# ArchDD/CPP-Raytracer-Rasterizer

Hardware: AMD Instinct MI355X
Metric: Mrays/s (primary+shadow) (higher is better)
Workload: dtype f32

## Files before the change

cpp-raytracer-rasterizer_amd/capi/binned.cpp:

```cpp
#include "capi.hpp"

namespace mirt {


int ensure_pairs(RtScratch &S, size_t cap)
{
    int r;
    if ((r = dev_realloc(&S.d_entries, cap)) || (r = dev_realloc(&S.d_pair_keys, cap)) || (r = dev_realloc(&S.d_pair_vals, cap)) ||
        (r = dev_realloc(&S.d_sorted_keys, cap)) || (r = dev_realloc(&S.d_tmp_vals, cap))) { S.cap_entries = 0; return r; }
    S.cap_entries = (uint32_t)cap;
    return MIRT_OK;
}

constexpr uint32_t BIN_MAX_KEYS = BUCKET_SORT_MAX_BUCKETS * 1024u - 1u;

void poll_pair_count(RtScratch &S)
{
    if (S.count_pending && hipEventQuery(S.ev_count) == hipSuccess) {
        S.known_pairs = *S.h_count; S.have_known = true; S.count_pending = false;
    }
    (void)hipGetLastError();
}

int bin_pass(RtScratch &S, BinSet bs, const OriginRow *cam_tab, const OriginRow *light_tab, uint32_t *counter, uint32_t *bin_off,
             bool fresh, uint32_t *npairs, bool may_guess = false)
{
    int rc;
    poll_pair_count(S);
    if (!fresh && may_guess && S.have_known && S.known_pairs > S.cap_used) fresh = true;
    const bool guess = fresh && may_guess && S.have_known;
    if (!S.d_entries || !S.cap_entries) {
        static const size_t initial = [] { const long v = env_int("MIRT_BIN_INITIAL_PAIRS", 0); return v > 0 ? (size_t)v : (size_t)1 << 20; }();
        if ((rc = ensure_pairs(S, initial))) return rc;
    }
    if (bs.nbins > BIN_MAX_KEYS) return fail(MIRT_ERR_INVALID_ARGUMENT, "binning: %u sort keys exceed the %u the bucket sort holds", bs.nbins, BIN_MAX_KEYS);
    bs.chunk_tris = 256;
    const dim3 bin_grid((unsigned)std::min<long long>((long long)((g.n + bs.chunk_tris - 1) / bs.chunk_tris) * bs.nframes, (long long)g.cu_count * 8));
    bs.counters = counter;
    const uint32_t nbuckets = bucket_sort_buckets(bs.nbins);
    if (nbuckets + 1 > S.cap_buckets) {
        S.cap_buckets = 0;
        if ((rc = dev_realloc(&S.d_bucket, (size_t)3 * (nbuckets + 1)))) return rc;
        HIP_TRY(hipMemsetAsync(S.d_bucket, 0, sizeof(uint32_t) * 3 * (nbuckets + 1), g.stream));
        S.cap_buckets = nbuckets + 1;
        S.bucket_dirty = false;
    }
    uint32_t *bcnt = S.d_bucket, *bbase = S.d_bucket + S.cap_buckets, *bcur = S.d_bucket + 2 * (size_t)S.cap_buckets;
    bs.bucket_cnt = bcnt; bs.nbuckets = nbuckets; bs.bucket_shift = bucket_sort_shift(bs.nbins);
    const size_t bin_lds = (size_t)nbuckets * sizeof(uint32_t);
    {
        static const bool once = [] {
            (void)hipFuncSetAttribute(reinterpret_cast<const void *>(&k_bin_pairs<512>), hipFuncAttributeMaxDynamicSharedMemorySize, 48 * 1024);
// ... 328 lines not shown
    const uint32_t cam_keys = (uint32_t)bs.frame0.nbu * (uint32_t)band_tile_rows * (uint32_t)bs.frame0.nshell;
    const int tshells = transient ? light_shells_for(nlights, cube_bins, 0u) : 1;
    const uint32_t per_light = 6u * (uint32_t)(cube_bins * cube_bins) * (uint32_t)tshells;
    bs.nbins = cam_keys;
    if (bs.nbins + 1 > S.cap_bins) {
        const size_t cap = (size_t)bs.nbins + 1;
        HIP_TRY(hipStreamSynchronize(g.stream));
        if ((rc = dev_realloc(&S.d_bin_off, cap))) { S.cap_bins = 0; return rc; }
        S.cap_bins = (uint32_t)cap;
        S.bin_key_valid = false;
    }
    if (!S.d_bin_counters) { HIP_TRY(hipMalloc(reinterpret_cast<void **>(&S.d_bin_counters), 512)); HIP_TRY(hipMemsetAsync(S.d_bin_counters, 0, 512, g.stream)); }
    if (S.sel_n != g.n) {
        HIP_TRY(hipStreamSynchronize(g.stream));
        S.sel_n = 0;
        if ((rc = dev_realloc(&S.d_sel, (size_t)g.n))) return rc;
        S.sel_n = g.n;
        S.bin_key_valid = false;
    }
    bs.bin_off = S.d_bin_off;

    uint64_t key = 0xcbf29ce484222325ull ^ g.scene_version;
    {
        auto mix = [&](const void *p, size_t nb) { const unsigned char *b = (const unsigned char *)p; for (size_t i = 0; i < nb; i++) { key ^= b[i]; key *= 0x100000001b3ull; } };
        mix(view, sizeof *view); mix(&y0, 4); mix(&y1, 4); mix(&g.n, 4); mix(&g.aa, 4);
    }
    const int bin_mode = 0;
    StreamState &ss = g.cur();
    ss.hits_clean[ss.hits_tog] = false;
    if (!S.d_frames) HIP_TRY(hipMalloc(reinterpret_cast<void **>(&S.d_frames), sizeof(BinFrameDesc) * (1 + 6 * MIRT_MAX_LIGHTS)));
    poll_pair_count(S);
// ... 20 lines not shown
        rc = transient_light_pass(L, f, origins, nlights, cube_bins, tshells, per_light, lkey, &lights_kept, reuse ? g.d_hits : nullptr);
        g.stream = main_stream;
        if (rc) return rc;
        if (forked) HIP_TRY(hipEventRecord(ss.ev_join, ss.aux));
    }
    if (reuse) {
        if (!(transient && !lights_kept)) HIP_TRY(hipMemsetAsync(g.d_hits, 0, HIT_BYTES, g.stream));
        g.stats.bins_reused = 1;
    } else {
        S.sel_parity ^= 1;
        SelectOut so;
        memset(&so, 0, sizeof so);
        so.cam_tab = S.d_cam_tab; so.sel = S.d_sel;
        so.sel_count = S.d_bin_counters + SEL_COUNT0 + S.sel_parity; so.sel_count_next = S.d_bin_counters + SEL_COUNT0 + (S.sel_parity ^ 1);
        so.zero_hits = g.d_hits; so.zero_counter = S.d_bin_counters;
        if ((rc = hist_prepare(S, bs.frame0, &so))) return rc;
        const unsigned sel_grid = (unsigned)std::min<long long>(((long long)g.n + 1023) / 1024, (long long)g.cu_count);
        hipLaunchKernelGGL(k_prep_select, dim3(sel_grid), dim3(1024), 0, g.stream, g.d_tris, g.n, bs.frame0, so);
        if ((rc = hist_publish(S))) return rc;
        bs.sel = S.d_sel; bs.sel_count = so.sel_count;
        g.stats_sel_count = so.sel_count;
        if ((rc = bin_pass(S, bs, S.d_cam_tab, nullptr, S.d_bin_counters, S.d_bin_off, true, &S.bin_entries, may_guess))) return rc;
        S.last_bin_mode = bin_mode;
        S.bin_key = key;
        S.bin_key_valid = true;
        if ((size_t)order_seg > S.cap_order) {
            HIP_TRY(hipStreamSynchronize(g.stream));
            S.cap_order = 0;
            if ((rc = dev_realloc(&S.d_order, (size_t)ORDER_GROUPS * ORDER_CLASSES * order_seg))) return rc;
            S.cap_order = order_seg;
        }
        hipLaunchKernelGGL(k_tile_order, dim3((pairs_x + 63) / 64, (unsigned)(bs.frame0.j1 - bs.frame0.j0)), dim3(64), 0, g.stream, cam_off, bs.frame0.nshell,
                           bs.frame0.nbu, bs.frame0.j0, bs.frame0.j1, S.d_bin_counters, S.cap_used, S.d_order, order_seg);
    }
    if (forked) HIP_TRY(hipStreamWaitEvent(g.stream, ss.ev_join, 0));
// ... 10 lines not shown
}

int hist_only_pass(const mirt_view *view)
{
    int rc;
    g.stream = g.cur().stream;
    RtScratch &S = g.cur().rt;
    if (S.cam_tab_n != g.n) {
        S.cam_tab_n = 0;
        if ((rc = dev_realloc(&S.d_cam_tab, (size_t)g.n))) return rc;
        S.cam_tab_n = g.n;
    }
    if (S.sel_n != g.n) {
        HIP_TRY(hipStreamSynchronize(g.stream));
        S.sel_n = 0;
        if ((rc = dev_realloc(&S.d_sel, (size_t)g.n))) return rc;
        S.sel_n = g.n;
    }
    if (!S.d_bin_counters) { HIP_TRY(hipMalloc(reinterpret_cast<void **>(&S.d_bin_counters), 512)); HIP_TRY(hipMemsetAsync(S.d_bin_counters, 0, 512, g.stream)); }
    S.bin_key_valid = false;
    const BinFrameDesc fr = make_camera_frame(view, 0, 0, g.aa);
    SelectOut so;
    memset(&so, 0, sizeof so);
    so.cam_tab = S.d_cam_tab; so.sel = S.d_sel;
    so.sel_count = S.d_bin_counters + HIST_SEL_COUNT; so.sel_count_next = S.d_bin_counters + HIST_SEL_COUNT + 1;
    if ((rc = hist_prepare(S, fr, &so))) return rc;
    if (!g.hist_armed) return MIRT_OK;
    HIP_TRY(hipMemsetAsync(so.sel_count, 0, 4, g.stream));
    const unsigned sel_grid = (unsigned)std::min<long long>(((long long)g.n + 1023) / 1024, (long long)g.cu_count);
    if (sel_grid) hipLaunchKernelGGL(k_prep_select, dim3(sel_grid), dim3(1024), 0, g.stream, g.d_tris, g.n, fr, so);
    HIP_TRY(hipGetLastError());
// ... 59 lines not shown
```

cpp-raytracer-rasterizer_amd/capi/capi.hpp:

```cpp
#pragma once

#include "../csrc/bin_sort.hpp"
#include "../csrc/comm.hpp"
#include "../csrc/cull.hpp"
#include "../csrc/dof.hpp"
#include "../csrc/rt_common.hpp"
#include "../csrc/raster_common.hpp"
#include "../csrc/rt_binned.hpp"
#include "../csrc/scan.hpp"
#include "env.hpp"

#include <cstdarg>
#include <cstdio>
#include <cstdlib>
#include <cstring>
#include <algorithm>
#include <cmath>
#include <vector>

#define MIRT_KERNEL __attribute__((global))

namespace mirt {

MIRT_KERNEL void k_prep_origin(const float *, int, const float *, v3, int, OriginRow *, OriginRow *, uint32_t *, unsigned long long *, uint32_t *);
// ... 49 lines not shown

extern char g_err[512];
int fail(int code, const char *fmt, ...);

#define HIP_TRY(expr)                                                                          \
    do {                                                                                       \
        hipError_t e_ = (expr);                                                                \
        if (e_ != hipSuccess)                                                                  \
            return fail(MIRT_ERR_HIP, "%s failed: %s (%s:%d)", #expr, hipGetErrorString(e_), __FILE__, __LINE__); \
    } while (0)

enum { EV_CALL0 = 0, EV_CALL1 = 1, EV_K0 = 2, EV_COUNT = 2 + 2 * 8 };
constexpr int MAX_FLIGHT = 4;
constexpr int SEL_COUNT0 = 80;
constexpr int HIST_SEL_COUNT = 82;
constexpr int HIST_RING = 4;
constexpr int HIST_SLOTS = HIST_RING + 1;
constexpr size_t HIT_BYTES = sizeof(unsigned long long) * HIT_SHARDS * HIT_SHARD_STRIDE;

struct RtScratch {
    OriginRow *d_cam_tab = nullptr;
    OriginRow *d_light_tab = nullptr;
    int cam_tab_n = 0, light_tab_n = 0, light_tab_lights = 0;
    float *d_origins = nullptr;
    uint32_t *d_flags = nullptr;
    BinFrameDesc *d_frames = nullptr;
    uint32_t *d_bin_off = nullptr, *d_bin_counters = nullptr;
    uint32_t *d_entries = nullptr;
    uint32_t *d_pair_keys = nullptr, *d_pair_vals = nullptr, *d_sorted_keys = nullptr;
    uint32_t *d_tmp_vals = nullptr;
// ... 279 lines not shown
```

cpp-raytracer-rasterizer_amd/csrc/rt_binned.hip:

```cpp
#include "rt_binned.hpp"

#include <float.h>

namespace mirt {

constexpr int BIN_L0 = BIN_COARSE * BIN_COARSE;

struct BinItem {
    float A0[4], A1[4], A2[4], Bu[4], Bv[4];
    float lou, hiu, lov, hiv;
};

__device__ __forceinline__ float bcastf(float v, int lane) { return __builtin_bit_cast(float, __builtin_amdgcn_readlane(__builtin_bit_cast(int, v), lane)); }

__device__ __forceinline__ float corner(float s, float lo, float hi) { return fmaxf(s * lo, s * hi); }

__device__ __forceinline__ bool cell_may_hit(const BinItem &u, const float (&A)[4], float I, float J, float K)
{
    bool ok = true;
#pragma unroll
    for (int k = 0; k < 4; k++) ok = ok && (__builtin_fmaf(J, u.Bv[k], __builtin_fmaf(I, u.Bu[k], A[k])) >= 0.0f);
    return ok && (I + K >= u.lou) && (I <= u.hiu) && (J + K >= u.lov) && (J <= u.hiv);
}

// ... 23 lines not shown
    for (int i = 0; i < 4; i++)
#pragma unroll
        for (int j = i + 1; j < 4; j++) {
#pragma unroll
            for (int k = j + 1; k < 4; k++) empty = empty || bin_triple_infeasible(G[i], G[j], G[k], U, V);
#pragma unroll
            for (int sd = 0; sd < 4; sd++) empty = empty || bin_triple_infeasible(G[i], G[j], side[sd], U, V);
        }
    return empty;
}

struct BinFrameGrid { int nbu, fj0, fj1, cells_x, cy0, ncell; uint32_t fbase, nshell; };

constexpr int BIN_PAIR_BUF = 4096;
constexpr int BIN_TESTS_PER_THREAD = 2;
constexpr int BIN_DIRECT_SIDE = 32;

struct BinLargeSink {
    uint32_t *s_keys, *s_vals;
    uint32_t *s_fill;
    uint32_t *s_valid;
    uint32_t *g_count;
    BinPairs out;
    uint32_t *bucket_cnt;
    int bucket_shift;
};

__device__ __forceinline__ void bin_walk_large(const BinItem &u, uint32_t utri, uint32_t ushell, const BinFrameGrid &gr, int lane,
                                               const BinLargeSink &sink, unsigned long long cells0)
{
// ... 45 lines not shown
            }
        }
    }
#ifdef MIRT_BIN_STATS
    if (lane == 0) {
        uint32_t *c = sink.g_count;
        atomicAdd(&c[2], 1u); atomicAdd(&c[3], dbg_l1); atomicAdd(&c[4], dbg_steps); atomicAdd(&c[5], dbg_pairs);
        atomicMax(&c[6], dbg_steps);
        if (dbg_steps > 100) atomicAdd(&c[7], 1u);
    }
#endif
}

constexpr int SEL_WG = 1024;
constexpr int SEL_STAGE = 8192;

__global__ __launch_bounds__(SEL_WG) void k_prep_select(const float *__restrict__ tris15, int n, const BinFrameDesc fr, const SelectOut out)
{
    __shared__ uint32_t s_hist[SEL_HIST_MAX];
    __shared__ uint32_t s_sel[SEL_STAGE];
    __shared__ uint32_t s_fill, s_base;
    const int lane = threadIdx.x & 63;
    if (blockIdx.x == 0) {
        if (out.zero_hits)
            for (int g = threadIdx.x; g < HIT_SHARDS * HIT_SHARD_STRIDE; g += SEL_WG) out.zero_hits[g] = 0ull;
        if (out.zero_counter && (threadIdx.x == 0 || (threadIdx.x >= 16 && threadIdx.x < 80))) out.zero_counter[threadIdx.x] = 0u;
        if (threadIdx.x == 0) *out.sel_count_next = 0u;
        if (out.zero_faces && (int)threadIdx.x < out.zero_faces_n) out.zero_faces[threadIdx.x] = 0u;
    }
    if (out.hist && threadIdx.x < SEL_HIST_MAX) s_hist[threadIdx.x] = 0u;
    if (threadIdx.x == 0) s_fill = 0u;
    __syncthreads();
    const v3 S = V3(fr.S[0], fr.S[1], fr.S[2]);
    const int nchunks = (n + SEL_WG - 1) / SEL_WG;
    const int hist_rows = ((fr.nbv - 1) >> out.hist_shift) + 1;
    auto flush = [&]() {
        __syncthreads();
        const uint32_t staged = s_fill;
        if (threadIdx.x == 0 && staged) s_base = atomicAdd(out.sel_count, staged);
        __syncthreads();
        const uint32_t base = s_base;
        for (uint32_t i = threadIdx.x; i < staged; i += SEL_WG) out.sel[base + i] = s_sel[i];
        __syncthreads();
        if (threadIdx.x == 0) s_fill = 0u;
        __syncthreads();
    };
    for (int c = blockIdx.x; c < nchunks; c += gridDim.x) {
        if (s_fill + (uint32_t)SEL_WG > (uint32_t)SEL_STAGE) flush();
        const int i = c * SEL_WG + (int)threadIdx.x;
        bool keep = false;
        OriginRow r;
        if (i < n) {
            const float *t15 = tris15 + (size_t)15 * i;
            r = make_origin_row(t15, S);
            PreBox box;
            bool boxed;
            keep = frame_may_see(r, ld3(t15), ld3(t15 + 3), ld3(t15 + 6), fr, &box, &boxed);
            if (out.hist && boxed) {
                const float flo_u = fmaxf(ceilf(box.lou) - 1.0f, 0.0f), fhi_u = fminf(floorf(box.hiu), (float)(fr.nbu - 1));
                const float flo_v = fmaxf(ceilf(box.lov) - 1.0f, 0.0f), fhi_v = fminf(floorf(box.hiv), (float)(fr.nbv - 1));
                if (flo_u <= fhi_u && flo_v <= fhi_v) {
                    const uint32_t wi = (uint32_t)((int)fhi_u - (int)flo_u + 1);
                    const int ja = (int)flo_v, jb = (int)fhi_v;
                    for (int cr = ja >> out.hist_shift; cr <= (jb >> out.hist_shift) && cr < hist_rows; cr++) {
                        const int lo = max(ja, cr << out.hist_shift), hi = min(jb, ((cr + 1) << out.hist_shift) - 1);
                        atomicAdd(&s_hist[cr], wi * (uint32_t)(hi - lo + 1));
                    }
                }
            }
            if (keep) out.cam_tab[i] = r;
        }
        const unsigned long long m = __builtin_amdgcn_ballot_w64(keep);
        if (m) {
            uint32_t at0 = 0;
            if (lane == 0) at0 = atomicAdd(&s_fill, (uint32_t)__popcll(m));
            at0 = (uint32_t)__builtin_amdgcn_readfirstlane((int)at0);
            if (keep) s_sel[at0 + (uint32_t)__popcll(m & ((1ull << lane) - 1ull))] = (uint32_t)i;
        }
        __syncthreads();
    }
    flush();
    if (out.hist && threadIdx.x < SEL_HIST_MAX) {
        const uint32_t v = s_hist[threadIdx.x];
        if (v && (int)threadIdx.x < hist_rows) atomicAdd(&out.hist[threadIdx.x], v);
    }
}

constexpr int FACE_STAGE = 2048;
__global__ __launch_bounds__(SEL_WG) void k_select_faces(const float *__restrict__ tris15, int n, const float *__restrict__ origins ,
                                                        const BinFrameDesc *__restrict__ faces , OriginRow *__restrict__ light_tab,
                                                        uint32_t *__restrict__ lists, uint32_t stride, uint32_t *__restrict__ face_counts)
{
// ... 58 lines not shown
                                                   const OriginRow *__restrict__ light_tab, int n, BinSet bs, BinPairs out)
{
    extern __shared__ uint32_t s_bucket[];
    __shared__ uint32_t s_keys[BIN_PAIR_BUF], s_vals[BIN_PAIR_BUF];
    __shared__ float4 s_A2[256], s_Bu[256], s_Bv[256], s_box[256];
    __shared__ uint32_t s_org[256];
    __shared__ uint32_t s_ni[256];
    __shared__ uint32_t s_tri[256];
    __shared__ uint32_t s_pre[257];
    __shared__ uint32_t s_wave[4];
    __shared__ uint32_t s_base, s_fill, s_valid;
    const int lane = threadIdx.x & 63, wave = threadIdx.x >> 6;
    const int chunk_tris = bs.chunk_tris;
    const int nchunks = (n + chunk_tris - 1) / chunk_tris;
    const bool listed = bs.sel != nullptr;
    const uint32_t nsel = listed ? min(*bs.sel_count, (uint32_t)n) : 0u;
    const int cam_chunk = (listed && nsel < 32768u) ? 64 : chunk_tris;
    const int ncam = listed ? (int)((nsel + (uint32_t)cam_chunk - 1u) / (uint32_t)cam_chunk) : 0;
    const int nrest = listed ? bs.nframes - 1 : bs.nframes;
    const bool faces_listed = bs.face_lists != nullptr;
    __shared__ uint32_t s_first[MAX_BIN_FRAMES + 1];
    if (faces_listed) {
        if (threadIdx.x == 0) {
            uint32_t run = 0;
            for (int ff = 0; ff < nrest; ff++) { s_first[ff] = run; run += (min(bs.face_counts[ff], (uint32_t)n) + (uint32_t)chunk_tris - 1u) / (uint32_t)chunk_tris; }
            s_first[nrest] = run;
        }
        __syncthreads();
    }
    const int nwork = ncam + (faces_listed ? (int)s_first[nrest] : nchunks * nrest);
    if (threadIdx.x == 0) { s_fill = 0u; s_valid = (uint32_t)BIN_PAIR_BUF; }
    if (bs.bucket_cnt)
        for (uint32_t b = threadIdx.x; b < bs.nbuckets; b += WG) s_bucket[b] = 0u;
// ... 34 lines not shown
        int chunk, frame;
        const uint32_t *list = nullptr;
        uint32_t nhere = (uint32_t)n;
        const bool from_cam_list = w < ncam;
        if (from_cam_list) { chunk = w; frame = 0; list = bs.sel; nhere = nsel; }
        else if (faces_listed) {
            const uint32_t w2 = (uint32_t)(w - ncam);
            int lo = 0, hi = nrest;
            while (hi - lo > 1) { const int mid = (lo + hi) >> 1; if (s_first[mid] <= w2) lo = mid; else hi = mid; }
            chunk = (int)(w2 - s_first[lo]);
            frame = lo + (listed ? 1 : 0);
            list = bs.face_lists + (size_t)lo * bs.face_stride;
            nhere = min(bs.face_counts[lo], (uint32_t)n);
        } else { const int w2 = w - ncam; chunk = w2 / nrest; frame = w2 - chunk * nrest + (listed ? 1 : 0); }
        const int item_tris = from_cam_list ? cam_chunk : chunk_tris;
        const uint32_t slot = (uint32_t)chunk * (uint32_t)item_tris + threadIdx.x;
        const uint32_t tri = ((int)threadIdx.x < item_tris && slot < nhere) ? (list ? list[slot] : slot) : 0xFFFFFFFFu;
        const BinFrameDesc fr = bs.frames ? bs.frames[frame] : bs.frame0;
        BinFrameGrid gr;
        gr.nbu = fr.nbu; gr.fj0 = fr.j0; gr.fj1 = fr.j1; gr.fbase = fr.base; gr.nshell = (uint32_t)max(fr.nshell, 1);
        gr.cells_x = (gr.nbu + BIN_L0 - 1) / BIN_L0; gr.cy0 = gr.fj0 / BIN_L0;
        gr.ncell = gr.cells_x * ((gr.fj1 + BIN_L0 - 1) / BIN_L0 - gr.cy0);
        const int nbu = gr.nbu, fj0 = gr.fj0, fj1 = gr.fj1;
        BinItem it;
        memset(&it, 0, sizeof it);
        int kind = 0;
#ifdef MIRT_BIN_STATS
        int dbg_state = 0;
#endif
        int i_lo = 0, i_hi = -1, j_lo = 0, j_hi = -1;
        unsigned long long cells = 0;
        uint32_t shell = 0;
        if (tri < (uint32_t)n && fj1 > fj0) {
            const OriginRow &row = (fr.tab == 0) ? cam_tab[tri] : light_tab[(size_t)(fr.tab - 1) * n + tri];
            shell = bin_shell_of(fr, row.r1.w);
            TriBinFns t = make_bin_fns(row, fr);
            add_bbox(t, tris15 + (size_t)15 * tri, fr);
#ifdef MIRT_BIN_STATS
// ... 3 lines not shown
            const bool both = fabsf(t.nb) < T || !(t.nb == t.nb);
            const float sgn = t.nb < 0.0f ? -1.0f : 1.0f;
            const EdgeFn *fn[4] = { &t.n, &t.p, &t.q, &t.s };
            const float inf = __builtin_huge_valf();
#pragma unroll
            for (int k = 0; k < 4; k++) {
                const float su = sgn * fn[k]->cu, sv = sgn * fn[k]->cv;
                const float base = sgn * fn[k]->c0 + fn[k]->m + su * fr.ulo + sv * fr.vlo;
                it.Bu[k] = both ? 0.0f : su * fr.du;
                it.Bv[k] = both ? 0.0f : sv * fr.dv;
                it.A0[k] = both ? inf : base + corner(su, fr.pad_lo, (float)BIN_L0 * fr.du + fr.pad_hi) + corner(sv, fr.pad_lo, (float)BIN_L0 * fr.dv + fr.pad_hi);
                it.A1[k] = both ? inf : base + corner(su, fr.pad_lo, (float)BIN_COARSE * fr.du + fr.pad_hi) + corner(sv, fr.pad_lo, (float)BIN_COARSE * fr.dv + fr.pad_hi);
                it.A2[k] = both ? inf : base + corner(su, fr.pad_lo, fr.du + fr.pad_hi) + corner(sv, fr.pad_lo, fr.dv + fr.pad_hi);
            }
            if (t.bstate == BOX_VALID) {
                it.lou = (t.bu0 - fr.ulo - fr.pad_hi) / fr.du; it.hiu = (t.bu1 - fr.ulo - fr.pad_lo) / fr.du;
                it.lov = (t.bv0 - fr.vlo - fr.pad_hi) / fr.dv; it.hiv = (t.bv1 - fr.vlo - fr.pad_lo) / fr.dv;
                it.lou -= 3.814697265625e-06f * (1.0f + fabsf(it.lou)); it.hiu += 3.814697265625e-06f * (1.0f + fabsf(it.hiu));
                it.lov -= 3.814697265625e-06f * (1.0f + fabsf(it.lov)); it.hiv += 3.814697265625e-06f * (1.0f + fabsf(it.hiv));
            } else if (t.bstate == BOX_EMPTY) {
                it.lou = it.lov = inf; it.hiu = it.hiv = -inf;
            } else {
                it.lou = it.lov = -inf; it.hiu = it.hiv = inf;
            }
            const float flo_u = fmaxf(ceilf(it.lou) - 1.0f, 0.0f), fhi_u = fminf(floorf(it.hiu), (float)(nbu - 1));
            const float flo_v = fmaxf(ceilf(it.lov) - 1.0f, (float)fj0), fhi_v = fminf(floorf(it.hiv), (float)(fj1 - 1));
            if (flo_u <= fhi_u && flo_v <= fhi_v) {
                i_lo = (int)flo_u; i_hi = (int)fhi_u; j_lo = (int)flo_v; j_hi = (int)fhi_v;
                kind = (i_hi - i_lo < BIN_DIRECT_SIDE && j_hi - j_lo < BIN_DIRECT_SIDE) ? 1 : 2;
            }
            if (kind == 2) {
                for (int c = 0; c < gr.ncell && c < 64; c++) {
                    const int cx = c % gr.cells_x, cy = gr.cy0 + c / gr.cells_x;
                    if (cell_may_hit(it, it.A0, (float)(cx * BIN_L0), (float)(cy * BIN_L0), (float)BIN_L0)) cells |= 1ull << c;
// ... 140 lines not shown
```

cpp-raytracer-rasterizer_amd/csrc/rt_binned.hpp:

```cpp
#pragma once

#include "rt_common.hpp"

namespace mirt {

#ifndef MIRT_ORDER_STRIPE_SHIFT
#define MIRT_ORDER_STRIPE_SHIFT 2
#endif
constexpr int ORDER_STRIPE_SHIFT = MIRT_ORDER_STRIPE_SHIFT;
constexpr int BIN_TILE = 8;
constexpr int BIN_COARSE = 8;
constexpr int CUBE_BINS_MIN = 64;
constexpr int MAX_BIN_FRAMES = 1 + 6 * MIRT_MAX_LIGHTS;

struct BinFrameDesc {
    float P0[3], Pu[3], Pv[3];
    float S[3];
    float ru[3], rv[3], rw[3];
    float ulo, vlo, du, dv;
    float pad_lo, pad_hi;
    float dmax;
    int nbu, nbv;
    int j0, j1;
    uint32_t base;
// ... 16 lines not shown
struct BinSet {
    const BinFrameDesc *frames;
    BinFrameDesc frame0;
    int nframes;
    uint32_t nbins;
    uint32_t *bin_off;
    uint32_t *entries;
    uint32_t cap_entries;
    uint32_t *counters;
    uint32_t *bucket_cnt;
    uint32_t nbuckets;
    int bucket_shift;
    int chunk_tris;
    const uint32_t *sel;
    const uint32_t *sel_count;
    const uint32_t *face_lists;
    const uint32_t *face_counts;
    uint32_t face_stride;
};

constexpr int SEL_HIST_MAX = 256;
struct SelectOut {
    OriginRow *cam_tab;
    uint32_t *sel;
    uint32_t *sel_count;
    uint32_t *sel_count_next;
    uint32_t *hist;
    int hist_shift;
    uint32_t *zero_faces;
    int zero_faces_n;
    unsigned long long *zero_hits;
    uint32_t *zero_counter;
};

struct BinPairs {
    uint32_t *keys;
    uint32_t *vals;
    uint32_t cap;
};

struct EdgeFn { float c0, cu, cv, m; };

__device__ __forceinline__ EdgeFn make_edge_fn(float gx, float gy, float gz, const BinFrameDesc &fr)
{
    EdgeFn e;
    e.c0 = gx * fr.P0[0] + gy * fr.P0[1] + gz * fr.P0[2];
    e.cu = gx * fr.Pu[0] + gy * fr.Pu[1] + gz * fr.Pu[2];
// ... 28 lines not shown

__device__ __forceinline__ void add_bbox(TriBinFns &t, const float *t15, const BinFrameDesc &fr)
{
    float us[3], vs[3], pad = 0.0f;
    int front = 0, behind = 0;
#pragma unroll
    for (int j = 0; j < 3; j++) {
        const float gx = fr.S[0] - t15[3 * j], gy = fr.S[1] - t15[3 * j + 1], gz = fr.S[2] - t15[3 * j + 2];
        const float w = fr.rw[0] * gx + fr.rw[1] * gy + fr.rw[2] * gz;
        const float wm = fabsf(fr.rw[0] * gx) + fabsf(fr.rw[1] * gy) + fabsf(fr.rw[2] * gz);
        front += (w > 0.00390625f * wm);
        behind += (w < -0.00390625f * wm);
        const float un = fr.ru[0] * gx + fr.ru[1] * gy + fr.ru[2] * gz, vn = fr.rv[0] * gx + fr.rv[1] * gy + fr.rv[2] * gz;
        const float um = fabsf(fr.ru[0] * gx) + fabsf(fr.ru[1] * gy) + fabsf(fr.ru[2] * gz);
        const float vm = fabsf(fr.rv[0] * gx) + fabsf(fr.rv[1] * gy) + fabsf(fr.rv[2] * gz);
        us[j] = un / w; vs[j] = vn / w;
        const float iw = 1.0f / fabsf(w);
        pad = fmaxf(pad, 4.76837158203125e-07f * ((um + fabsf(us[j]) * wm) * iw + (vm + fabsf(vs[j]) * wm) * iw) +
                             2.384185791015625e-07f * (fabsf(us[j]) + fabsf(vs[j])));
    }
    if (front != 3 && behind != 3) return;
    const float u0 = fminf(fminf(us[0], us[1]), us[2]), u1 = fmaxf(fmaxf(us[0], us[1]), us[2]);
    const float v0 = fminf(fminf(vs[0], vs[1]), vs[2]), v1 = fmaxf(fmaxf(vs[0], vs[1]), vs[2]);
    const float ext = fmaxf(u1 - u0, v1 - v0);
    const float ax = us[1] - us[0], ay = vs[1] - vs[0], bx = us[2] - us[0], by = vs[2] - vs[0], cx = us[2] - us[1], cy = vs[2] - vs[1];
    const float area2 = fabsf(ax * by - ay * bx);
    const float per = sqrtf(ax * ax + ay * ay) + sqrtf(bx * bx + by * by) + sqrtf(cx * cx + cy * cy);
    const float dp = t.p.m / sqrtf(t.p.cu * t.p.cu + t.p.cv * t.p.cv);
    const float dq = t.q.m / sqrtf(t.q.cu * t.q.cu + t.q.cv * t.q.cv);
    const float ds = t.s.m / sqrtf(t.s.cu * t.s.cu + t.s.cv * t.s.cv);
    const float d = fmaxf(fmaxf(dp, dq), ds) + pad;
    if (behind == 3) {
        const float area_lo = area2 - 2.0f * pad * per - 4.76837158203125e-07f * (fabsf(ax * by) + fabsf(ay * bx));
        if (d < 0.5f * (area_lo / per)) t.bstate = BOX_EMPTY;
        return;
    }
    const float l01 = sqrtf(ax * ax + ay * ay), l02 = sqrtf(bx * bx + by * by), l12 = sqrtf(cx * cx + cy * cy);
    const float e01x = ax / l01, e01y = ay / l01, e02x = bx / l02, e02y = by / l02, e12x = cx / l12, e12y = cy / l12;
    const float dd = 1.25f * d;
    const float k0 = dd / fabsf(e01x * e02y - e01y * e02x), k1 = dd / fabsf(e01x * e12y - e01y * e12x), k2 = dd / fabsf(e02x * e12y - e02y * e12x);
    const float px0 = us[0] - k0 * (e01x + e02x), py0 = vs[0] - k0 * (e01y + e02y);
    const float px1 = us[1] - k1 * (e12x - e01x), py1 = vs[1] - k1 * (e12y - e01y);
    const float px2 = us[2] + k2 * (e02x + e12x), py2 = vs[2] + k2 * (e02y + e12y);
    const float slack = 2.0f * pad + 1.0e-6f * ext;
    const float bu0 = fminf(fminf(px0, px1), px2) - slack, bu1 = fmaxf(fmaxf(px0, px1), px2) + slack;
    const float bv0 = fminf(fminf(py0, py1), py2) - slack, bv1 = fmaxf(fmaxf(py0, py1), py2) + slack;
    if (!(bu0 > -1.0e30f && bu1 < 1.0e30f && bv0 > -1.0e30f && bv1 < 1.0e30f)) return;
    t.bu0 = fminf(bu0, u0 - slack); t.bu1 = fmaxf(bu1, u1 + slack); t.bv0 = fminf(bv0, v0 - slack); t.bv1 = fmaxf(bv1, v1 + slack);
    t.bstate = BOX_VALID;
}

struct PreBox { float lou, hiu, lov, hiv; };
__device__ __forceinline__ bool frame_may_see(const OriginRow &row, v3 va, v3 vb, v3 vc, const BinFrameDesc &fr, PreBox *box, bool *boxed)
{
    *boxed = false;
    const float nbv = row.r0.w;
    if (!(fabsf(nbv) >= 1.6940658945086007e-21f)) return true;
    const v3 vert[3] = { va, vb, vc };
    float us[3], vs[3], pad = 0.0f;
// ... 99 lines not shown
```

cpp-raytracer-rasterizer_amd/csrc/rt_trace.hip:

```cpp
#include "rt_binned.hpp"

#include <float.h>

namespace mirt {


__global__ __launch_bounds__(256) void k_geo_table(const float *__restrict__ tris15, int n, GeoRow *__restrict__ geo, ShadeRow *__restrict__ shade)
{
    const int t = blockIdx.x * blockDim.x + threadIdx.x;
    if (t >= n) return;
    const float *t15 = tris15 + (size_t)15 * t;
    const v3 v0 = ld3(t15), e1 = sub3(ld3(t15 + 3), v0), e2 = sub3(ld3(t15 + 6), v0);
    GeoRow g;
    g.g0 = make_float4(v0.x, v0.y, v0.z, e1.x);
    g.g1 = make_float4(e1.y, e1.z, e2.x, e2.y);
    g.g2 = make_float4(e2.z, 0.0f, 0.0f, 0.0f);
    geo[t] = g;
    const v3 nd = normalize3(ld3(t15 + 9));
    ShadeRow sr;
    sr.n = make_float4(nd.x, nd.y, nd.z, 0.0f);
    sr.col = make_float4(t15[12], t15[13], t15[14], 0.0f);
    shade[t] = sr;
}

// ... 279 lines not shown
            const v3p nd = neg3p(mat3_mul_vecp(f.rot, d));

            s.best[lane] = MIN_T_NONE; s.best[lane + 64] = MIN_T_NONE;
            s.flag[lane] = 0; s.flag[lane + 64] = 0;
            if (STATS) ncand += nokA * nA + nokB * nB;
            float lbA = okA ? FLT_MAX : -__builtin_huge_valf(), lbB = okB ? FLT_MAX : -__builtin_huge_valf();
            float tbA = FLT_MAX, tbB = FLT_MAX;
            for (uint32_t base = 0; base < nmax; base += TR_STAGE) {
                const int cntA = (int)min((uint32_t)TR_STAGE, nA > base ? nA - base : 0u);
                const int cntB = (int)min((uint32_t)TR_STAGE, nB > base ? nB - base : 0u);
                wave_lds_fence();
                float my_near = 0.0f;
                const int sh = lane >> 4, sj = lane & 15;
                const bool stage = lane < 32 && sj < (sh ? cntB : cntA);
                if (stage) {
                    const uint32_t idx = brute ? tf.sel[base + (uint32_t)sj] : tf.cam_entries[(sh ? begB : begA) + base + (uint32_t)sj];
                    const float4 *src = reinterpret_cast<const float4 *>(f.cam_tab + idx);
                    const float4 a0 = src[0], a1 = src[1], a2 = src[2];
                    if (!lazy) {
                        const float4 *gsrc = geo4 + (size_t)idx * 3;
                        float4 *gdst = s.geo + lane * 3;
                        gdst[0] = gsrc[0]; gdst[1] = gsrc[1]; gdst[2] = gsrc[2];
                    }
                    float *dst = reinterpret_cast<float *>(s.rows) + sj * 24 + sh;
                    dst[0] = a0.x; dst[2] = a0.y; dst[4] = a0.z; dst[6] = a0.w;
                    dst[8] = a1.x; dst[10] = a1.y; dst[12] = a1.z; dst[14] = a1.w;
                    dst[16] = a2.x; dst[18] = a2.y; dst[20] = a2.z; dst[22] = __uint_as_float(idx);
                    my_near = a1.w;
                } else if (lane < 32) {
                    reinterpret_cast<float *>(s.rows)[sj * 24 + sh + 14] = __builtin_huge_valf();
                }
// ... 256 lines not shown
```

Before: 47520.

## Deal heavy-footprint triangles round-robin across binning work items, use fast rcp/rsq

The select kernel now flags triangles whose screen footprint spans many bins, or that have no box, and writes them to a second list. The binning kernel reserves one eighth of each camera work item for these heavy triangles, dealt round-robin across chunks, so expensive triangles no longer cluster in a few workgroups. Separately, divides and sqrts in the box computation are replaced with hardware rcp/rsq/sqrt intrinsics. The error margins are widened to keep the bounds conservative. This adds a second atomic-compacted list and extra sel memory, and carries a small risk that the looser bounds produce more pairs.

Result: no change. 47060 (-1.0%).

```diff
diff --git a/cpp-raytracer-rasterizer_amd/capi/binned.cpp b/cpp-raytracer-rasterizer_amd/capi/binned.cpp
--- a/cpp-raytracer-rasterizer_amd/capi/binned.cpp
+++ b/cpp-raytracer-rasterizer_amd/capi/binned.cpp
@@ -35,7 +35,8 @@
     }
     if (bs.nbins > BIN_MAX_KEYS) return fail(MIRT_ERR_INVALID_ARGUMENT, "binning: %u sort keys exceed the %u the bucket sort holds", bs.nbins, BIN_MAX_KEYS);
     bs.chunk_tris = 256;
-    const dim3 bin_grid((unsigned)std::min<long long>((long long)((g.n + bs.chunk_tris - 1) / bs.chunk_tris) * bs.nframes, (long long)g.cu_count * 8));
+    const int item_tris = bs.heavy ? bs.chunk_tris - (bs.chunk_tris >> 3) : bs.chunk_tris;
+    const dim3 bin_grid((unsigned)std::min<long long>((long long)((g.n + item_tris - 1) / item_tris) * bs.nframes, (long long)g.cu_count * 8));
     bs.counters = counter;
     const uint32_t nbuckets = bucket_sort_buckets(bs.nbins);
     if (nbuckets + 1 > S.cap_buckets) {
@@ -394,7 +395,7 @@
     if (S.sel_n != g.n) {
         HIP_TRY(hipStreamSynchronize(g.stream));
         S.sel_n = 0;
-        if ((rc = dev_realloc(&S.d_sel, (size_t)g.n))) return rc;
+        if ((rc = dev_realloc(&S.d_sel, (size_t)2 * g.n))) return rc;
         S.sel_n = g.n;
         S.bin_key_valid = false;
     }
@@ -445,11 +446,17 @@
         so.cam_tab = S.d_cam_tab; so.sel = S.d_sel;
         so.sel_count = S.d_bin_counters + SEL_COUNT0 + S.sel_parity; so.sel_count_next = S.d_bin_counters + SEL_COUNT0 + (S.sel_parity ^ 1);
         so.zero_hits = g.d_hits; so.zero_counter = S.d_bin_counters;
+        static const bool deal = env_int("MIRT_BIN_DEAL", 1) != 0;
+        if (deal) {
+            so.heavy = S.d_sel + g.n;
+            so.heavy_count = S.d_bin_counters + HEAVY_COUNT0 + S.sel_parity; so.heavy_count_next = S.d_bin_counters + HEAVY_COUNT0 + (S.sel_parity ^ 1);
+        }
         if ((rc = hist_prepare(S, bs.frame0, &so))) return rc;
         const unsigned sel_grid = (unsigned)std::min<long long>(((long long)g.n + 1023) / 1024, (long long)g.cu_count);
         hipLaunchKernelGGL(k_prep_select, dim3(sel_grid), dim3(1024), 0, g.stream, g.d_tris, g.n, bs.frame0, so);
         if ((rc = hist_publish(S))) return rc;
         bs.sel = S.d_sel; bs.sel_count = so.sel_count;
+        bs.heavy = so.heavy; bs.heavy_count = so.heavy_count;
         g.stats_sel_count = so.sel_count;
         if ((rc = bin_pass(S, bs, S.d_cam_tab, nullptr, S.d_bin_counters, S.d_bin_off, true, &S.bin_entries, may_guess))) return rc;
         S.last_bin_mode = bin_mode;
@@ -490,7 +497,7 @@
     if (S.sel_n != g.n) {
         HIP_TRY(hipStreamSynchronize(g.stream));
         S.sel_n = 0;
-        if ((rc = dev_realloc(&S.d_sel, (size_t)g.n))) return rc;
+        if ((rc = dev_realloc(&S.d_sel, (size_t)2 * g.n))) return rc;
         S.sel_n = g.n;
     }
     if (!S.d_bin_counters) { HIP_TRY(hipMalloc(reinterpret_cast<void **>(&S.d_bin_counters), 512)); HIP_TRY(hipMemsetAsync(S.d_bin_counters, 0, 512, g.stream)); }
diff --git a/cpp-raytracer-rasterizer_amd/capi/capi.hpp b/cpp-raytracer-rasterizer_amd/capi/capi.hpp
--- a/cpp-raytracer-rasterizer_amd/capi/capi.hpp
+++ b/cpp-raytracer-rasterizer_amd/capi/capi.hpp
@@ -87,6 +87,7 @@
 constexpr int MAX_FLIGHT = 4;
 constexpr int SEL_COUNT0 = 80;
 constexpr int HIST_SEL_COUNT = 82;
+constexpr int HEAVY_COUNT0 = 84;
 constexpr int HIST_RING = 4;
 constexpr int HIST_SLOTS = HIST_RING + 1;
 constexpr size_t HIT_BYTES = sizeof(unsigned long long) * HIT_SHARDS * HIT_SHARD_STRIDE;
diff --git a/cpp-raytracer-rasterizer_amd/csrc/rt_binned.hip b/cpp-raytracer-rasterizer_amd/csrc/rt_binned.hip
--- a/cpp-raytracer-rasterizer_amd/csrc/rt_binned.hip
+++ b/cpp-raytracer-rasterizer_amd/csrc/rt_binned.hip
@@ -61,6 +61,7 @@
 
 constexpr int BIN_PAIR_BUF = 4096;
 constexpr int BIN_TESTS_PER_THREAD = 2;
+constexpr int BIN_DEAL_SHIFT = 3;
 constexpr int BIN_DIRECT_SIDE = 32;
 
 struct BinLargeSink {
@@ -136,48 +137,59 @@
 
 constexpr int SEL_WG = 1024;
 constexpr int SEL_STAGE = 8192;
+constexpr int SEL_HEAVY_STAGE = 2048;
 
 __global__ __launch_bounds__(SEL_WG) void k_prep_select(const float *__restrict__ tris15, int n, const BinFrameDesc fr, const SelectOut out)
 {
     __shared__ uint32_t s_hist[SEL_HIST_MAX];
     __shared__ uint32_t s_sel[SEL_STAGE];
-    __shared__ uint32_t s_fill, s_base;
+    __shared__ uint32_t s_hvy[SEL_HEAVY_STAGE];
+    __shared__ uint32_t s_fill, s_base, s_hfill, s_hbase;
     const int lane = threadIdx.x & 63;
     if (blockIdx.x == 0) {
         if (out.zero_hits)
             for (int g = threadIdx.x; g < HIT_SHARDS * HIT_SHARD_STRIDE; g += SEL_WG) out.zero_hits[g] = 0ull;
         if (out.zero_counter && (threadIdx.x == 0 || (threadIdx.x >= 16 && threadIdx.x < 80))) out.zero_counter[threadIdx.x] = 0u;
         if (threadIdx.x == 0) *out.sel_count_next = 0u;
+        if (threadIdx.x == 0 && out.heavy) *out.heavy_count_next = 0u;
         if (out.zero_faces && (int)threadIdx.x < out.zero_faces_n) out.zero_faces[threadIdx.x] = 0u;
     }
     if (out.hist && threadIdx.x < SEL_HIST_MAX) s_hist[threadIdx.x] = 0u;
-    if (threadIdx.x == 0) s_fill = 0u;
+    if (threadIdx.x == 0) { s_fill = 0u; s_hfill = 0u; }
     __syncthreads();
     const v3 S = V3(fr.S[0], fr.S[1], fr.S[2]);
     const int nchunks = (n + SEL_WG - 1) / SEL_WG;
     const int hist_rows = ((fr.nbv - 1) >> out.hist_shift) + 1;
     auto flush = [&]() {
         __syncthreads();
-        const uint32_t staged = s_fill;
+        const uint32_t staged = s_fill, hstaged = s_hfill;
         if (threadIdx.x == 0 && staged) s_base = atomicAdd(out.sel_count, staged);
-        __syncthreads();
-        const uint32_t base = s_base;
+        if (threadIdx.x == 64 && hstaged) s_hbase = atomicAdd(out.heavy_count, hstaged);
+        __syncthreads();
+        const uint32_t base = s_base, hbase = s_hbase;
         for (uint32_t i = threadIdx.x; i < staged; i += SEL_WG) out.sel[base + i] = s_sel[i];
-        __syncthreads();
-        if (threadIdx.x == 0) s_fill = 0u;
+        for (uint32_t i = threadIdx.x; i < hstaged; i += SEL_WG) out.heavy[hbase + i] = s_hvy[i];
+        __syncthreads();
+        if (threadIdx.x == 0) { s_fill = 0u; s_hfill = 0u; }
         __syncthreads();
     };
     for (int c = blockIdx.x; c < nchunks; c += gridDim.x) {
-        if (s_fill + (uint32_t)SEL_WG > (uint32_t)SEL_STAGE) flush();
+        if (s_fill + (uint32_t)SEL_WG > (uint32_t)SEL_STAGE || s_hfill + (uint32_t)SEL_WG > (uint32_t)SEL_HEAVY_STAGE) flush();
         const int i = c * SEL_WG + (int)threadIdx.x;
-        bool keep = false;
+        bool keep = false, heavy = false;
         OriginRow r;
         if (i < n) {
             const float *t15 = tris15 + (size_t)15 * i;
             r = make_origin_row(t15, S);
-            PreBox box;
+            PreBox box = { 0.0f, 0.0f, 0.0f, 0.0f };
             bool boxed;
             keep = frame_may_see(r, ld3(t15), ld3(t15 + 3), ld3(t15 + 6), fr, &box, &boxed);
+            if (keep) out.cam_tab[i] = r;
+            if (out.heavy) {
+                const float wu = fminf(floorf(box.hiu), (float)(fr.nbu - 1)) - fmaxf(ceilf(box.lou) - 1.0f, 0.0f) + 1.0f;
+                const float wv = fminf(floorf(box.hiv), (float)(fr.j1 - 1)) - fmaxf(ceilf(box.lov) - 1.0f, (float)fr.j0) + 1.0f;
+                heavy = keep && (!boxed || (wu > 0.0f && wv > 0.0f && wu * wv > BIN_HEAVY_BINS));
+            }
             if (out.hist && boxed) {
                 const float flo_u = fmaxf(ceilf(box.lou) - 1.0f, 0.0f), fhi_u = fminf(floorf(box.hiu), (float)(fr.nbu - 1));
                 const float flo_v = fmaxf(ceilf(box.lov) - 1.0f, 0.0f), fhi_v = fminf(floorf(box.hiv), (float)(fr.nbv - 1));
@@ -190,14 +202,20 @@
                     }
                 }
             }
-            if (keep) out.cam_tab[i] = r;
         }
         const unsigned long long m = __builtin_amdgcn_ballot_w64(keep);
         if (m) {
             uint32_t at0 = 0;
             if (lane == 0) at0 = atomicAdd(&s_fill, (uint32_t)__popcll(m));
             at0 = (uint32_t)__builtin_amdgcn_readfirstlane((int)at0);
-            if (keep) s_sel[at0 + (uint32_t)__popcll(m & ((1ull << lane) - 1ull))] = (uint32_t)i;
+            if (keep) s_sel[at0 + (uint32_t)__popcll(m & ((1ull << lane) - 1ull))] = (uint32_t)i | (heavy ? SEL_HEAVY_BIT : 0u);
+        }
+        const unsigned long long mh = __builtin_amdgcn_ballot_w64(heavy);
+        if (mh) {
+            uint32_t at0 = 0;
+            if (lane == 0) at0 = atomicAdd(&s_hfill, (uint32_t)__popcll(mh));
+            at0 = (uint32_t)__builtin_amdgcn_readfirstlane((int)at0);
+            if (heavy) s_hvy[at0 + (uint32_t)__popcll(mh & ((1ull << lane) - 1ull))] = (uint32_t)i;
         }
         __syncthreads();
     }
@@ -286,9 +304,14 @@
     const int chunk_tris = bs.chunk_tris;
     const int nchunks = (n + chunk_tris - 1) / chunk_tris;
     const bool listed = bs.sel != nullptr;
-    const uint32_t nsel = listed ? min(*bs.sel_count, (uint32_t)n) : 0u;
+    const bool deal = listed && bs.heavy != nullptr;
+    const uint32_t *const second_count = deal ? bs.heavy_count : bs.sel_count;
+    const uint32_t sel_raw = listed ? *bs.sel_count : 0u, heavy_raw = listed ? *second_count : 0u;
+    const uint32_t nsel = min(sel_raw, (uint32_t)n);
     const int cam_chunk = (listed && nsel < 32768u) ? 64 : chunk_tris;
-    const int ncam = listed ? (int)((nsel + (uint32_t)cam_chunk - 1u) / (uint32_t)cam_chunk) : 0;
+    const uint32_t nheavy = deal ? min(heavy_raw, nsel) : 0u;
+    const int cam_res = deal ? cam_chunk >> BIN_DEAL_SHIFT : 0, cam_ord = cam_chunk - cam_res;
+    const int ncam = listed ? (int)max((nsel + (uint32_t)cam_ord - 1u) / (uint32_t)cam_ord, deal ? (nheavy + (uint32_t)cam_res - 1u) / (uint32_t)cam_res : 0u) : 0;
     const int nrest = listed ? bs.nframes - 1 : bs.nframes;
     const bool faces_listed = bs.face_lists != nullptr;
     __shared__ uint32_t s_first[MAX_BIN_FRAMES + 1];
@@ -353,14 +376,24 @@
             nhere = min(bs.face_counts[lo], (uint32_t)n);
         } else { const int w2 = w - ncam; chunk = w2 / nrest; frame = w2 - chunk * nrest + (listed ? 1 : 0); }
         const int item_tris = from_cam_list ? cam_chunk : chunk_tris;
-        const uint32_t slot = (uint32_t)chunk * (uint32_t)item_tris + threadIdx.x;
-        const uint32_t tri = ((int)threadIdx.x < item_tris && slot < nhere) ? (list ? list[slot] : slot) : 0xFFFFFFFFu;
+        uint32_t tri = 0xFFFFFFFFu;
+        if (from_cam_list && deal) {
+            const int hl = (int)threadIdx.x - cam_ord;
+            const uint32_t slot = (uint32_t)chunk * (uint32_t)cam_ord + threadIdx.x;
+            const uint32_t hslot = (uint32_t)chunk + (uint32_t)max(hl, 0) * (uint32_t)ncam;
+            if (hl < 0) { if (slot < nsel) tri = bs.sel[slot]; }
+            else if (hl < cam_res && hslot < nheavy) tri = bs.heavy[hslot];
+        } else {
+            const uint32_t slot = (uint32_t)chunk * (uint32_t)item_tris + threadIdx.x;
+            if ((int)threadIdx.x < item_tris && slot < nhere) tri = list ? list[slot] & SEL_INDEX_MASK : slot;
+        }
         const BinFrameDesc fr = bs.frames ? bs.frames[frame] : bs.frame0;
         BinFrameGrid gr;
         gr.nbu = fr.nbu; gr.fj0 = fr.j0; gr.fj1 = fr.j1; gr.fbase = fr.base; gr.nshell = (uint32_t)max(fr.nshell, 1);
         gr.cells_x = (gr.nbu + BIN_L0 - 1) / BIN_L0; gr.cy0 = gr.fj0 / BIN_L0;
         gr.ncell = gr.cells_x * ((gr.fj1 + BIN_L0 - 1) / BIN_L0 - gr.cy0);
         const int nbu = gr.nbu, fj0 = gr.fj0, fj1 = gr.fj1;
+        const float idu = __builtin_amdgcn_rcpf(fr.du), idv = __builtin_amdgcn_rcpf(fr.dv);
         BinItem it;
         memset(&it, 0, sizeof it);
         int kind = 0;
@@ -394,10 +427,10 @@
                 it.A2[k] = both ? inf : base + corner(su, fr.pad_lo, fr.du + fr.pad_hi) + corner(sv, fr.pad_lo, fr.dv + fr.pad_hi);
             }
             if (t.bstate == BOX_VALID) {
-                it.lou = (t.bu0 - fr.ulo - fr.pad_hi) / fr.du; it.hiu = (t.bu1 - fr.ulo - fr.pad_lo) / fr.du;
-                it.lov = (t.bv0 - fr.vlo - fr.pad_hi) / fr.dv; it.hiv = (t.bv1 - fr.vlo - fr.pad_lo) / fr.dv;
-                it.lou -= 3.814697265625e-06f * (1.0f + fabsf(it.lou)); it.hiu += 3.814697265625e-06f * (1.0f + fabsf(it.hiu));
-                it.lov -= 3.814697265625e-06f * (1.0f + fabsf(it.lov)); it.hiv += 3.814697265625e-06f * (1.0f + fabsf(it.hiv));
+                it.lou = (t.bu0 - fr.ulo - fr.pad_hi) * idu; it.hiu = (t.bu1 - fr.ulo - fr.pad_lo) * idu;
+                it.lov = (t.bv0 - fr.vlo - fr.pad_hi) * idv; it.hiv = (t.bv1 - fr.vlo - fr.pad_lo) * idv;
+                it.lou -= 7.62939453125e-06f * (1.0f + fabsf(it.lou)); it.hiu += 7.62939453125e-06f * (1.0f + fabsf(it.hiu));
+                it.lov -= 7.62939453125e-06f * (1.0f + fabsf(it.lov)); it.hiv += 7.62939453125e-06f * (1.0f + fabsf(it.hiv));
             } else if (t.bstate == BOX_EMPTY) {
                 it.lou = it.lov = inf; it.hiu = it.hiv = -inf;
             } else {
diff --git a/cpp-raytracer-rasterizer_amd/csrc/rt_binned.hpp b/cpp-raytracer-rasterizer_amd/csrc/rt_binned.hpp
--- a/cpp-raytracer-rasterizer_amd/csrc/rt_binned.hpp
+++ b/cpp-raytracer-rasterizer_amd/csrc/rt_binned.hpp
@@ -54,12 +54,17 @@
     int chunk_tris;
     const uint32_t *sel;
     const uint32_t *sel_count;
+    const uint32_t *heavy;
+    const uint32_t *heavy_count;
     const uint32_t *face_lists;
     const uint32_t *face_counts;
     uint32_t face_stride;
 };
 
 constexpr int SEL_HIST_MAX = 256;
+constexpr uint32_t SEL_HEAVY_BIT = 0x80000000u;
+constexpr uint32_t SEL_INDEX_MASK = 0x7FFFFFFFu;
+constexpr float BIN_HEAVY_BINS = 512.0f;
 struct SelectOut {
     OriginRow *cam_tab;
     uint32_t *sel;
@@ -71,6 +76,9 @@
     int zero_faces_n;
     unsigned long long *zero_hits;
     uint32_t *zero_counter;
+    uint32_t *heavy;
+    uint32_t *heavy_count;
+    uint32_t *heavy_count_next;
 };
 
 struct BinPairs {
@@ -129,35 +137,40 @@
         const float un = fr.ru[0] * gx + fr.ru[1] * gy + fr.ru[2] * gz, vn = fr.rv[0] * gx + fr.rv[1] * gy + fr.rv[2] * gz;
         const float um = fabsf(fr.ru[0] * gx) + fabsf(fr.ru[1] * gy) + fabsf(fr.ru[2] * gz);
         const float vm = fabsf(fr.rv[0] * gx) + fabsf(fr.rv[1] * gy) + fabsf(fr.rv[2] * gz);
-        us[j] = un / w; vs[j] = vn / w;
-        const float iw = 1.0f / fabsf(w);
-        pad = fmaxf(pad, 4.76837158203125e-07f * ((um + fabsf(us[j]) * wm) * iw + (vm + fabsf(vs[j]) * wm) * iw) +
-                             2.384185791015625e-07f * (fabsf(us[j]) + fabsf(vs[j])));
+        const float iw = __builtin_amdgcn_rcpf(w);
+        us[j] = un * iw; vs[j] = vn * iw;
+        const float aiw = fabsf(iw);
+        pad = fmaxf(pad, 4.76837158203125e-07f * ((um + fabsf(us[j]) * wm) * aiw + (vm + fabsf(vs[j]) * wm) * aiw) +
+                             4.76837158203125e-07f * (fabsf(us[j]) + fabsf(vs[j])));
     }
     if (front != 3 && behind != 3) return;
     const float u0 = fminf(fminf(us[0], us[1]), us[2]), u1 = fmaxf(fmaxf(us[0], us[1]), us[2]);
     const float v0 = fminf(fminf(vs[0], vs[1]), vs[2]), v1 = fmaxf(fmaxf(vs[0], vs[1]), vs[2]);
     const float ext = fmaxf(u1 - u0, v1 - v0);
     const float ax = us[1] - us[0], ay = vs[1] - vs[0], bx = us[2] - us[0], by = vs[2] - vs[0], cx = us[2] - us[1], cy = vs[2] - vs[1];
-    const float area2 = fabsf(ax * by - ay * bx);
-    const float per = sqrtf(ax * ax + ay * ay) + sqrtf(bx * bx + by * by) + sqrtf(cx * cx + cy * cy);
-    const float dp = t.p.m / sqrtf(t.p.cu * t.p.cu + t.p.cv * t.p.cv);
-    const float dq = t.q.m / sqrtf(t.q.cu * t.q.cu + t.q.cv * t.q.cv);
-    const float ds = t.s.m / sqrtf(t.s.cu * t.s.cu + t.s.cv * t.s.cv);
-    const float d = fmaxf(fmaxf(dp, dq), ds) + pad;
+    const float dp = t.p.m * __builtin_amdgcn_rsqf(t.p.cu * t.p.cu + t.p.cv * t.p.cv);
+    const float dq = t.q.m * __builtin_amdgcn_rsqf(t.q.cu * t.q.cu + t.q.cv * t.q.cv);
+    const float ds = t.s.m * __builtin_amdgcn_rsqf(t.s.cu * t.s.cu + t.s.cv * t.s.cv);
+    const float d = fmaxf(fmaxf(dp, dq), ds) * 1.0000019073486328125f + pad;
+    const float q01 = ax * ax + ay * ay, q02 = bx * bx + by * by, q12 = cx * cx + cy * cy;
     if (behind == 3) {
+        const float area2 = fabsf(ax * by - ay * bx);
+        const float per = (__builtin_amdgcn_sqrtf(q01) + __builtin_amdgcn_sqrtf(q02) + __builtin_amdgcn_sqrtf(q12)) * 1.00000095367431640625f;
         const float area_lo = area2 - 2.0f * pad * per - 4.76837158203125e-07f * (fabsf(ax * by) + fabsf(ay * bx));
-        if (d < 0.5f * (area_lo / per)) t.bstate = BOX_EMPTY;
+        if (d < 0.5f * (area_lo * __builtin_amdgcn_rcpf(per) * 0.99999809265136719f)) t.bstate = BOX_EMPTY;
         return;
     }
-    const float l01 = sqrtf(ax * ax + ay * ay), l02 = sqrtf(bx * bx + by * by), l12 = sqrtf(cx * cx + cy * cy);
-    const float e01x = ax / l01, e01y = ay / l01, e02x = bx / l02, e02y = by / l02, e12x = cx / l12, e12y = cy / l12;
-    const float dd = 1.25f * d;
-    const float k0 = dd / fabsf(e01x * e02y - e01y * e02x), k1 = dd / fabsf(e01x * e12y - e01y * e12x), k2 = dd / fabsf(e02x * e12y - e02y * e12x);
+    const float r01 = __builtin_amdgcn_rsqf(q01), r02 = __builtin_amdgcn_rsqf(q02), r12 = __builtin_amdgcn_rsqf(q12);
+    const float e01x = ax * r01, e01y = ay * r01, e02x = bx * r02, e02y = by * r02, e12x = cx * r12, e12y = cy * r12;
+    const float dd = 1.2500047683715820f * d;
+    const float s0 = fmaxf(fabsf(e01x * e02y - e01y * e02x) - 1.9073486328125e-06f, 0.0f);
+    const float s1 = fmaxf(fabsf(e01x * e12y - e01y * e12x) - 1.9073486328125e-06f, 0.0f);
+    const float s2 = fmaxf(fabsf(e02x * e12y - e02y * e12x) - 1.9073486328125e-06f, 0.0f);
+    const float k0 = dd * __builtin_amdgcn_rcpf(s0), k1 = dd * __builtin_amdgcn_rcpf(s1), k2 = dd * __builtin_amdgcn_rcpf(s2);
     const float px0 = us[0] - k0 * (e01x + e02x), py0 = vs[0] - k0 * (e01y + e02y);
     const float px1 = us[1] - k1 * (e12x - e01x), py1 = vs[1] - k1 * (e12y - e01y);
     const float px2 = us[2] + k2 * (e02x + e12x), py2 = vs[2] + k2 * (e02y + e12y);
-    const float slack = 2.0f * pad + 1.0e-6f * ext;
+    const float slack = 2.0f * pad + 1.0e-6f * ext + 1.9073486328125e-06f * fmaxf(fmaxf(k0, k1), k2);
     const float bu0 = fminf(fminf(px0, px1), px2) - slack, bu1 = fmaxf(fmaxf(px0, px1), px2) + slack;
     const float bv0 = fminf(fminf(py0, py1), py2) - slack, bv1 = fmaxf(fmaxf(py0, py1), py2) + slack;
     if (!(bu0 > -1.0e30f && bu1 < 1.0e30f && bv0 > -1.0e30f && bv1 < 1.0e30f)) return;
diff --git a/cpp-raytracer-rasterizer_amd/csrc/rt_trace.hip b/cpp-raytracer-rasterizer_amd/csrc/rt_trace.hip
--- a/cpp-raytracer-rasterizer_amd/csrc/rt_trace.hip
+++ b/cpp-raytracer-rasterizer_amd/csrc/rt_trace.hip
@@ -317,7 +317,7 @@
                 const int sh = lane >> 4, sj = lane & 15;
                 const bool stage = lane < 32 && sj < (sh ? cntB : cntA);
                 if (stage) {
-                    const uint32_t idx = brute ? tf.sel[base + (uint32_t)sj] : tf.cam_entries[(sh ? begB : begA) + base + (uint32_t)sj];
+                    const uint32_t idx = brute ? (tf.sel[base + (uint32_t)sj] & SEL_INDEX_MASK) : tf.cam_entries[(sh ? begB : begA) + base + (uint32_t)sj];
                     const float4 *src = reinterpret_cast<const float4 *>(f.cam_tab + idx);
                     const float4 a0 = src[0], a1 = src[1], a2 = src[2];
                     if (!lazy) {
```
